# FintanH/rust-crdt

Hardware: AMD Instinct MI355X
Metric: replica-merges/sec (whole node) + achieved HBM GB/s as % of MI355X peak (higher is better)
Workload: dtype u64

## Files before the change

### rust-crdt_amd/csrc/common.hpp

```cpp
#pragma once

#include <hip/hip_runtime.h>

#include <cstdint>
#include <cstdio>
#include <algorithm>
#include <cstring>
#include <map>
#include <string>
#include <vector>

#include "crdt_gpu.h"
#include "shard_host.hpp"

namespace crdt {

using u64 = unsigned long long;
using u64x2 = unsigned long long __attribute__((ext_vector_type(2)));

constexpr int kWave = 64;

#ifndef CRDT_APPLY_WPE
#define CRDT_APPLY_WPE 0
#endif
// ... 36 lines not shown
  int map_lazyv = 1;
  int map_st = 0;
  int shagree = 0;
  int map_diag = 0;
  int rows_blocks_per_cu = 0;
  int apply_hot_slots = 8;
  int map_apply_hot = 1 << 20;
  int map_forget_vec2 = 1;
  int map_pair_reg = 1;
  int pair_rows = 256;
  int pair_ur = 8;
  int pair_occ = 1;
  int map_forget_bpc = 1;
  int mvreg_forget_bpc = 32;
  int map_pair_pf = 0;
  int map_pair_nt = 1;
  int map_pair_bpc = 64;
  int merge_flat = 1;
  int merge_flat_u = 2;
  int merge_ppl = 8;
  int stage_kb = 262144;
  int wire_walk = 1;
  int wire_fill = 1;
  int host_stream = 1;
  int apply_lane = 1;
  int apply_fence = 0;
  int orswot_apply_pf = 0;
  int orswot_apply_stg = 0;
  int orswot_apply_l2pf = 0;
  int orswot_apply_meta = 1;
  int orswot_apply_hpf = 0;
  int map_counter_dma = 0;
  int map_counter_depth = 8;
  int map_counter_kpw = 0;
  int map_counter_cs = 1;
  int map_counter_cl = 0;
  int map_orswot_cs = 0;
  int map_orswot_wide = 0;
  int map_nested_lds = 1;
  int map_apply_meta = 1;
  int map_apply_pf = 1;
  int read_bpc = 0;
  int read_unroll = 8;
  int read_nt = 1;
  int eqv_ppl = 8;
  int eqv_bpc = 32;
};

struct PendingTiming {
  std::string name;
  hipEvent_t start, stop;
};

}

struct crdt_ctx {
  int device = 0;
  hipStream_t stream = nullptr;
  int cu_count = 256;
  bool timing = false;
  crdt::Tune tune;
  std::string last_error;
  void *scratch = nullptr;
  size_t scratch_bytes = 0;
  void *dscratch = nullptr;
  size_t dscratch_bytes = 0;
  unsigned *counters = nullptr;
  size_t counters_n = 0;
  void *pinned = nullptr;
  size_t pinned_bytes = 0;
  hipEvent_t pinned_done = nullptr;
  std::map<std::string, crdt::KernelTimer> timers;
  std::vector<crdt::PendingTiming> pending;
  std::vector<hipEvent_t> free_events;
  void *comm = nullptr;
  int nranks = 1, rank = 0;
  void (*comm_destroy)(void *) = nullptr;
  void *sbuf[8] = {};
  size_t sbuf_bytes[8] = {};
  bool has_ops = false;
  crdt_comm_ops ops{};
  hipStream_t astream = nullptr;
  hipEvent_t a_main = nullptr, a_done = nullptr;
  void *a_dev = nullptr, *a_host = nullptr;
  size_t a_rows = 0;
  std::string comm_note;
  void (*comm_release)(crdt_ctx *) = nullptr;
  crdt::shard_host::PlanCache plans;
  bool chk_pending = false;
  uint64_t chk_key = 0;
  void *chk_dev = nullptr;
  uint64_t *chk_host = nullptr;
  hipEvent_t chk_ev = nullptr;
  int (*comm_check)(crdt_ctx *) = nullptr;
  int mem_kind = CRDT_MEM_DEVICE;
  hipStream_t hstream = nullptr;
  void *hbuf[2] = {};
  size_t hbuf_bytes = 0;
  void *hacc = nullptr;
  size_t hacc_bytes = 0;
  hipEvent_t hcopied[2] = {}, hfree[2] = {};
};

namespace crdt {

int fail(crdt_ctx *ctx, int code, const char *fmt, ...);
int hip_fail(crdt_ctx *ctx, hipError_t e, const char *what);
int ensure_scratch(crdt_ctx *ctx, size_t bytes);
int ensure_dscratch(crdt_ctx *ctx, size_t bytes);
int ensure_counters(crdt_ctx *ctx, size_t n);
int stage_h2d(crdt_ctx *ctx, void *dst, const void *src, size_t bytes);
int device_fill(crdt_ctx *ctx, void *dst, size_t bytes, unsigned char byte);
void timing_begin(crdt_ctx *ctx, const char *name);
void timing_end(crdt_ctx *ctx);
void timing_add_host(crdt_ctx *ctx, const char *name, double ms);

struct DefPlan {
  const size_t *def_off;
  unsigned long long G, D, M, A, Mw;
  const u64 *def_clock, *def_members;
  const u64 *out_clock;
  u64 *out_entries;
  int apply_ceiling;
  u64 *hash;
  unsigned *surv;
  unsigned *nsurv;
  uint8_t *out_keep;
  u64 *out_members;
  u64 *tkey;
  unsigned *trep;
  unsigned long long tmask;
};
int launch_deferred(crdt_ctx *ctx, const size_t *host_def_off, DefPlan q, const u64 *dev_def_off = nullptr,
                    unsigned *status = nullptr);
int stage_def_off_dev(crdt_ctx *ctx, const u64 *src, size_t *dst, size_t G, size_t D, unsigned *status,
                      unsigned *flags);

enum class Op : int { Max = 0, Or = 1 };

template <Op OP>
__device__ __forceinline__ u64 join(u64 a, u64 b) {
  if constexpr (OP == Op::Max) return a > b ? a : b;
  else return a | b;
}
template <Op OP>
__device__ __forceinline__ u64x2 join2(u64x2 a, u64x2 b) {
  u64x2 r;
  r.x = join<OP>(a.x, b.x);
  r.y = join<OP>(a.y, b.y);
  return r;
}

int lattice_lub_many(crdt_ctx *ctx, Op op, const u64 *in, size_t G, size_t R, size_t W,
                     size_t row_stride, size_t group_stride, u64 *out, size_t out_stride,
                     unsigned flags);
int lattice_merge_batch(crdt_ctx *ctx, Op op, u64 *self, const u64 *other, size_t N, size_t W,
                        size_t self_stride, size_t other_stride);
struct LubReq {
  Op op;
  const u64 *in;
  size_t G, R, W, row_stride, group_stride;
  u64 *out;
  size_t out_stride;
  unsigned flags;
};
int lattice_lub_many_multi(crdt_ctx *ctx, const LubReq *reqs, size_t n);
int lub_reqs_from_segments(crdt_ctx *ctx, const crdt_lub_segment *segs, size_t nseg, std::vector<LubReq> &reqs);

int lattice_lub_many_host(crdt_ctx *ctx, Op op, const u64 *in, size_t G, size_t R, size_t W,
                          size_t row_stride, size_t group_stride, u64 *out, size_t out_stride,
                          unsigned flags);
int lattice_merge_batch_host(crdt_ctx *ctx, Op op, u64 *self, const u64 *other, size_t N, size_t W,
                             size_t self_stride, size_t other_stride);
int lww_lub_many_dev(crdt_ctx *ctx, const u64 *marker, const u64 *val, size_t G, size_t R, size_t group_stride,
                     u64 *out_marker, u64 *out_val, u64 *first_conflict, unsigned flags);
int lww_merge_batch_dev(crdt_ctx *ctx, u64 *sm, u64 *sv, const u64 *om, const u64 *ov, size_t N, uint8_t *conflict);
int lww_lub_many_host(crdt_ctx *ctx, const u64 *marker, const u64 *val, size_t G, size_t R, size_t group_stride,
                      u64 *out_marker, u64 *out_val, u64 *first_conflict, unsigned flags);
int lww_merge_batch_host(crdt_ctx *ctx, u64 *sm, u64 *sv, const u64 *om, const u64 *ov, size_t N, uint8_t *conflict);
int orswot_lub_many_host(crdt_ctx *ctx, const crdt_orswot_batch *in, crdt_orswot_out *out);
struct OrswotJoinExtra {
  const u64 *init_clock = nullptr, *init_entries = nullptr;
  unsigned *viol = nullptr;
};
int orswot_lub_many_ex(crdt_ctx *ctx, const crdt_orswot_batch *in, crdt_orswot_out *out, const OrswotJoinExtra &ex);
int orswot_merge_batch_host(crdt_ctx *ctx, const crdt_orswot_states *self, const crdt_orswot_states *other,
                            uint32_t *status);
// ... 57 lines not shown
```

### rust-crdt_amd/csrc/ctx.cpp

```cpp
#include <cstdarg>
#include <cstdlib>

#include "common.hpp"

namespace crdt {

static thread_local std::string g_orphan_error;

int fail(crdt_ctx *ctx, int code, const char *fmt, ...) {
  char buf[512];
  va_list ap;
  va_start(ap, fmt);
  vsnprintf(buf, sizeof buf, fmt, ap);
  va_end(ap);
  if (ctx) ctx->last_error = buf;
  else g_orphan_error = buf;
  return code;
}

int hip_fail(crdt_ctx *ctx, hipError_t e, const char *what) {
  return fail(ctx, CRDT_EHIP, "%s failed: %s (%d)", what, hipGetErrorString(e), (int)e);
}

int ensure_scratch(crdt_ctx *ctx, size_t bytes) {
// ... 2 lines not shown
    (void)hipStreamSynchronize(ctx->stream);
    (void)hipFree(ctx->scratch);
    ctx->scratch = nullptr;
    ctx->scratch_bytes = 0;
  }
  size_t want = bytes < (1u << 20) ? (1u << 20) : bytes + bytes / 4;
  hipError_t e = hipMalloc(&ctx->scratch, want);
  if (e != hipSuccess) {
    ctx->scratch = nullptr;
    return fail(ctx, CRDT_ENOMEM, "scratch hipMalloc(%zu) failed: %s", want, hipGetErrorString(e));
  }
  ctx->scratch_bytes = want;
  return CRDT_OK;
}

int ensure_dscratch(crdt_ctx *ctx, size_t bytes) {
  if (bytes <= ctx->dscratch_bytes) return CRDT_OK;
  if (ctx->dscratch) {
    (void)hipStreamSynchronize(ctx->stream);
    (void)hipFree(ctx->dscratch);
    ctx->dscratch = nullptr;
    ctx->dscratch_bytes = 0;
  }
  size_t want = bytes < (1u << 16) ? (1u << 16) : bytes + bytes / 4;
  hipError_t e = hipMalloc(&ctx->dscratch, want);
  if (e != hipSuccess) {
    ctx->dscratch = nullptr;
    return fail(ctx, CRDT_ENOMEM, "dscratch hipMalloc(%zu) failed: %s", want, hipGetErrorString(e));
  }
  ctx->dscratch_bytes = want;
  return CRDT_OK;
}

int ensure_counters(crdt_ctx *ctx, size_t n) {
  if (n <= ctx->counters_n) return CRDT_OK;
  if (ctx->counters) {
    (void)hipStreamSynchronize(ctx->stream);
    (void)hipFree(ctx->counters);
    ctx->counters = nullptr;
    ctx->counters_n = 0;
  }
  size_t want = n < 16384 ? 16384 : n * 2;
  hipError_t e = hipMalloc(&ctx->counters, want * sizeof(unsigned));
  if (e != hipSuccess) {
    ctx->counters = nullptr;
    return fail(ctx, CRDT_ENOMEM, "counter hipMalloc failed: %s", hipGetErrorString(e));
  }
  ctx->counters_n = want;
  return device_fill(ctx, ctx->counters, want * sizeof(unsigned), 0);
}

int stage_h2d(crdt_ctx *ctx, void *dst, const void *src, size_t bytes) {
  if (bytes == 0) return CRDT_OK;
  if (ctx->pinned_done) {
    hipError_t e = hipEventSynchronize(ctx->pinned_done);
    if (e != hipSuccess) return hip_fail(ctx, e, "hipEventSynchronize(pinned)");
  } else {
    hipError_t e = hipEventCreateWithFlags(&ctx->pinned_done, hipEventDisableTiming);
    if (e != hipSuccess) return hip_fail(ctx, e, "hipEventCreate(pinned)");
  }
  if (bytes > ctx->pinned_bytes) {
    if (ctx->pinned) (void)hipHostFree(ctx->pinned);
    ctx->pinned = nullptr;
    ctx->pinned_bytes = 0;
    size_t want = bytes < 65536 ? 65536 : bytes * 2;
    hipError_t e = hipHostMalloc(&ctx->pinned, want, hipHostMallocDefault);
    if (e != hipSuccess) return fail(ctx, CRDT_ENOMEM, "hipHostMalloc(%zu) failed", want);
    ctx->pinned_bytes = want;
  }
  std::memcpy(ctx->pinned, src, bytes);
  hipError_t e = hipMemcpyAsync(dst, ctx->pinned, bytes, hipMemcpyHostToDevice, ctx->stream);
  if (e != hipSuccess) return hip_fail(ctx, e, "hipMemcpyAsync(staged)");
  e = hipEventRecord(ctx->pinned_done, ctx->stream);
  if (e != hipSuccess) return hip_fail(ctx, e, "hipEventRecord(pinned)");
  return CRDT_OK;
}

__global__ void fill_u64_kernel(unsigned long long *p, size_t n, unsigned long long v) {
  for (size_t i = (size_t)blockIdx.x * blockDim.x + threadIdx.x; i < n; i += (size_t)gridDim.x * blockDim.x)
    p[i] = v;
}
__global__ void fill_u8_kernel(unsigned char *p, size_t n, unsigned char v) {
  for (size_t i = (size_t)blockIdx.x * blockDim.x + threadIdx.x; i < n; i += (size_t)gridDim.x * blockDim.x)
    p[i] = v;
}

int device_fill(crdt_ctx *ctx, void *dst, size_t bytes, unsigned char byte) {
  if (bytes == 0) return CRDT_OK;
  const bool wide = (reinterpret_cast<uintptr_t>(dst) % 8 == 0) && bytes % 8 == 0;
  const size_t n = wide ? bytes / 8 : bytes;
  size_t blocks = (n + kBlock - 1) / kBlock;
  const size_t cap = (size_t)ctx->cu_count * 8;
  if (blocks > cap) blocks = cap;
  if (wide)
    hipLaunchKernelGGL(fill_u64_kernel, dim3((unsigned)blocks), dim3(kBlock), 0, ctx->stream,
                       (unsigned long long *)dst, n, 0x0101010101010101ULL * byte);
  else
    hipLaunchKernelGGL(fill_u8_kernel, dim3((unsigned)blocks), dim3(kBlock), 0, ctx->stream,
                       (unsigned char *)dst, n, byte);
  hipError_t e = hipGetLastError();
  return e == hipSuccess ? CRDT_OK : hip_fail(ctx, e, "device_fill");
}

static hipEvent_t take_event(crdt_ctx *ctx) {
  if (!ctx->free_events.empty()) {
    hipEvent_t e = ctx->free_events.back();
    ctx->free_events.pop_back();
    return e;
  }
  hipEvent_t e = nullptr;
  (void)hipEventCreate(&e);
  return e;
}

void timing_begin(crdt_ctx *ctx, const char *name) {
  if (!ctx->timing) return;
  PendingTiming p;
  p.name = name;
  p.start = take_event(ctx);
  p.stop = take_event(ctx);
  (void)hipEventRecord(p.start, ctx->stream);
  ctx->pending.push_back(p);
}

void timing_end(crdt_ctx *ctx) {
  if (!ctx->timing || ctx->pending.empty()) return;
  (void)hipEventRecord(ctx->pending.back().stop, ctx->stream);
}

void timing_add_host(crdt_ctx *ctx, const char *name, double ms) {
  if (!ctx->timing) return;
  auto &t = ctx->timers[name];
  t.total_ms += ms;
  t.launches += 1;
}

static void drain_timings(crdt_ctx *ctx) {
  for (auto &p : ctx->pending) {
    (void)hipEventSynchronize(p.stop);
    float ms = 0.f;
    if (hipEventElapsedTime(&ms, p.start, p.stop) == hipSuccess) {
      auto &t = ctx->timers[p.name];
      t.total_ms += ms;
      t.launches += 1;
    }
    ctx->free_events.push_back(p.start);
    ctx->free_events.push_back(p.stop);
  }
  ctx->pending.clear();
}

}

using namespace crdt;
// ... 68 lines not shown
      else if (k == "hot" && v >= 0 && v <= 64) ctx->tune.apply_hot_slots = v;
      else if (k == "mhot" && v >= 0) ctx->tune.map_apply_hot = v;
      else if (k == "mfv2") ctx->tune.map_forget_vec2 = v != 0;
      else if (k == "stage_kb" && v >= 4) ctx->tune.stage_kb = v;
      else if (k == "mpreg" && v >= 0 && v <= 2) ctx->tune.map_pair_reg = v;
      else if (k == "prows" && (v == 64 || v == 128 || v == 256)) ctx->tune.pair_rows = v;
      else if (k == "pur" && (v == 2 || v == 4 || v == 8)) ctx->tune.pair_ur = v;
      else if (k == "pocc" && v >= 0 && v <= 8) ctx->tune.pair_occ = v;
      else if (k == "mppl" && v >= 1 && v <= 64) ctx->tune.merge_ppl = v;
      else if (k == "mflat" && v >= 0 && v <= 16) ctx->tune.merge_flat = v;
      else if (k == "mpbpc" && v >= 1 && v <= 4096) ctx->tune.map_pair_bpc = v;
      else if (k == "mfbpc" && v >= 1 && v <= 64) ctx->tune.map_forget_bpc = v;
      else if (k == "mvfbpc" && v >= 1 && v <= 64) ctx->tune.mvreg_forget_bpc = v;
      else if (k == "eqvppl" && v >= 1 && v <= 64) ctx->tune.eqv_ppl = v;
      else if (k == "eqvbpc" && v >= 1 && v <= 4096) ctx->tune.eqv_bpc = v;
    }
    pos = end + 1;
  }
}

int crdt_ctx_create(int device, crdt_ctx **out) {
  if (!out) return fail(nullptr, CRDT_EINVAL, "crdt_ctx_create: out is NULL");
  *out = nullptr;
  int n = 0;
  hipError_t e = hipGetDeviceCount(&n);
  if (e != hipSuccess || n == 0)
    return fail(nullptr, CRDT_EHIP, "crdt_ctx_create: no HIP device (%s)", hipGetErrorString(e));
  if (device < 0 || device >= n)
    return fail(nullptr, CRDT_EINVAL, "crdt_ctx_create: device %d out of range [0,%d)", device, n);
  e = hipSetDevice(device);
  if (e != hipSuccess) return hip_fail(nullptr, e, "hipSetDevice");
  auto *ctx = new crdt_ctx();
  ctx->device = device;
  hipDeviceProp_t prop;
  if (hipGetDeviceProperties(&prop, device) == hipSuccess && prop.multiProcessorCount > 0)
    ctx->cu_count = prop.multiProcessorCount;
  if (const char *t = getenv("CRDT_TUNE")) apply_tune(ctx, t);
  *out = ctx;
  return CRDT_OK;
}

int crdt_ctx_destroy(crdt_ctx *ctx) {
  if (!ctx) return CRDT_OK;
  (void)hipSetDevice(ctx->device);
  (void)hipStreamSynchronize(ctx->stream);
  for (auto &p : ctx->pending) {
    (void)hipEventDestroy(p.start);
    (void)hipEventDestroy(p.stop);
  }
  for (auto e : ctx->free_events) (void)hipEventDestroy(e);
  if (ctx->scratch) (void)hipFree(ctx->scratch);
  if (ctx->counters) (void)hipFree(ctx->counters);
  if (ctx->dscratch) (void)hipFree(ctx->dscratch);
  if (ctx->pinned) (void)hipHostFree(ctx->pinned);
  if (ctx->pinned_done) (void)hipEventDestroy(ctx->pinned_done);
  free_stage(ctx);
  if (ctx->comm && ctx->comm_destroy) ctx->comm_destroy(ctx->comm);
  if (ctx->comm_release) ctx->comm_release(ctx);
  for (void *b : ctx->sbuf)
    if (b) (void)hipFree(b);
  delete ctx;
  return CRDT_OK;
}

int crdt_ctx_set_stream(crdt_ctx *ctx, void *hip_stream) {
  CRDT_CHECK_CTX(ctx);
  ctx->stream = reinterpret_cast<hipStream_t>(hip_stream);
  return CRDT_OK;
}

int crdt_ctx_synchronize(crdt_ctx *ctx) {
  CRDT_CHECK_CTX(ctx);
  CRDT_HIP(ctx, hipSetDevice(ctx->device));
  CRDT_HIP(ctx, hipStreamSynchronize(ctx->stream));
  if (ctx->comm_check) return ctx->comm_check(ctx);
  return CRDT_OK;
}

const char *crdt_last_error(const crdt_ctx *ctx) {
  return ctx ? ctx->last_error.c_str() : g_orphan_error.c_str();
}

const char *crdt_version(void) { return "0.8.0"; }
int crdt_abi_version(void) { return CRDT_ABI_VERSION; }
const char *crdt_build_target(void) { return "gfx950"; }

int crdt_ctx_set_timing(crdt_ctx *ctx, int enable) {
  CRDT_CHECK_CTX(ctx);
  ctx->timing = enable != 0;
  return CRDT_OK;
}

int crdt_ctx_timing(crdt_ctx *ctx, const char *name, double *total_ms, uint64_t *launches) {
  CRDT_CHECK_CTX(ctx);
  if (!name) return fail(ctx, CRDT_EINVAL, "crdt_ctx_timing: name is NULL");
  drain_timings(ctx);
  auto it = ctx->timers.find(name);
  if (total_ms) *total_ms = it == ctx->timers.end() ? 0.0 : it->second.total_ms;
  if (launches) *launches = it == ctx->timers.end() ? 0 : it->second.launches;
  return CRDT_OK;
}

int crdt_ctx_timing_reset(crdt_ctx *ctx) {
  CRDT_CHECK_CTX(ctx);
  drain_timings(ctx);
  ctx->timers.clear();
  return CRDT_OK;
}
// ... 10 lines not shown
```

### rust-crdt_amd/csrc/map.hip

```cpp
#include <type_traits>

#include "common.hpp"

namespace crdt {

struct MapPlan {
  const u64 *clock;
  long long c_rs, c_gs;
  const u64 *ec;
  long long e_rs, e_gs;
  const u64 *vclk;
  long long vc_rs, vc_gs;
  const u64 *vval;
  long long vv_rs, vv_gs;
  const size_t *def_off;
  const unsigned *def_row;
  const u64 *def_clock;
  const u64 *def_keys;
  unsigned long long G, R, K, A, V, Kw, Vout;
  u64 *o_clock, *o_ec, *o_vclk, *o_vval;
  unsigned *o_nval;
  unsigned *o_flags;
  int spec;
  int nt;
// ... 2161 lines not shown
  if (R > 0 && (!in->clock || !in->ec || (V > 0 && (!in->vclk || !in->vval))))
    return fail(ctx, CRDT_EINVAL, "map_lub_many: NULL input");
  const bool wide = A > 256 || V > 8;
  if (Vout > 64) return fail(ctx, CRDT_EUNSUPPORTED, "map_lub_many: Vout = %zu > 64", Vout);
  const bool deep = out->Vstate > 16;
  if (out->Vstate > 64) return fail(ctx, CRDT_EUNSUPPORTED, "map_lub_many: Vstate = %zu > 64", out->Vstate);
  if (deep && map_deep_lds(out->Vstate, A) > 160 * 1024)
    return fail(ctx, CRDT_EUNSUPPORTED, "map_lub_many: Vstate = %zu values of A = %zu actors need %zu bytes of LDS (> 160 KiB)",
                out->Vstate, A, map_deep_lds(out->Vstate, A));
  if (G * K > 0x7fffffffULL) return fail(ctx, CRDT_EUNSUPPORTED, "map_lub_many: G*K too large");
  if (R > 0xfffffffeULL) return fail(ctx, CRDT_EUNSUPPORTED, "map_lub_many: R too large");
  const size_t D = doff ? Ddev : (in->def_off && G > 0) ? in->def_off[G] - in->def_off[0] : 0;
  if (in->def_off && in->def_off[0] != 0) return fail(ctx, CRDT_EINVAL, "map_lub_many: def_off[0] must be 0");
  if (D > 0 && (!in->def_row || !in->def_clock || !in->def_keys || !out->def_keep || !out->def_keys))
    return fail(ctx, CRDT_EINVAL, "map_lub_many: deferred buffers missing");
  if (D > 0xffffffffULL) return fail(ctx, CRDT_EUNSUPPORTED, "map_lub_many: too many deferred");
  CRDT_HIP(ctx, hipSetDevice(ctx->device));
  const size_t Kw = (K + 63) / 64;
  const size_t want = !deep && out->Vstate > Vout ? out->Vstate : Vout;

  MapPlan p{};
  p.clock = (const u64 *)in->clock;
  p.c_rs = in->clock_rstride;
  p.c_gs = in->clock_gstride;
  p.ec = (const u64 *)in->ec;
  p.e_rs = in->ec_rstride;
  p.e_gs = in->ec_gstride;
  p.vclk = (const u64 *)in->vclk;
  p.vc_rs = in->vclk_rstride;
  p.vc_gs = in->vclk_gstride;
  p.vval = (const u64 *)in->vval;
  p.vv_rs = in->vval_rstride;
  p.vv_gs = in->vval_gstride;
  p.G = G;
  p.R = R;
  p.K = K;
  p.A = A;
  p.V = V;
  p.Kw = Kw;
  p.Vout = Vout;
  p.o_clock = (u64 *)out->clock;
  p.o_ec = (u64 *)out->ec;
  p.o_vclk = (u64 *)out->vclk;
  p.o_vval = (u64 *)out->vval;
  p.o_nval = out->nval;
  p.o_flags = out->flags;
  p.spec = ctx->tune.map_spec;
  p.nt = ctx->tune.map_nt;
  p.scan2 = ctx->tune.map_scan2 && A % 2 == 0;
  p.scan3 = ctx->tune.map_scan3;
  p.lazyv = ctx->tune.map_lazyv;
  p.batch = ctx->tune.map_batch;
  p.diag = ctx->tune.map_diag;
  if (int rc = device_fill(ctx, out->flags, G * sizeof(unsigned), 0)) return rc;
  const bool even = ((p.c_rs | p.c_gs | p.e_rs | p.e_gs | p.vc_rs | p.vc_gs) & 1) == 0;
  const bool glds = !wide && ctx->tune.map_glds && R > 0 && A <= 64 && (A & 1) == 0 && (V == 1 || V == 2) &&
                    want <= 4 && even && aligned16(p.clock) && aligned16(p.ec) && aligned16(p.vclk) &&
                    G * ((R + 7) / 8) < 0x7fffffffULL;
  const bool rs = glds && ctx->tune.map_rs && A <= 32;
  const unsigned gC = (!rs && ctx->tune.map_chunk == 8 && ctx->tune.map_ring == 4) ? 8 : 16;
  const size_t off_b = D > 0 || doff ? ((G + 1) * sizeof(size_t) + 255) / 256 * 256 : 0;
  if (glds) p.nch = (R + gC - 1) / gC;
  p.st = rs && ctx->tune.map_st && A == 32 && V == 2 && !(ctx->tune.map_sh && K % 4 == 0);
  const size_t cm_b = glds ? G * p.nch * A * sizeof(u64) : 0;
  const size_t cm_pad = (cm_b + 15) / 16 * 16, nv_b = deep && !out->nval ? G * K * sizeof(unsigned) : 0;
  if (off_b + cm_pad + nv_b > 0)
    if (int rc = ensure_scratch(ctx, off_b + cm_pad + nv_b)) return rc;
  crdt_map_out dout = *out;
  if (deep) {
    if (!dout.nval) dout.nval = reinterpret_cast<uint32_t *>(static_cast<char *>(ctx->scratch) + off_b + cm_pad);
    p.o_nval = map_deep_tag(dout.nval);
  }
  if (doff && D == 0)
    if (int rc = stage_def_off_dev(ctx, doff, (size_t *)ctx->scratch, G, 0, nullptr, out->flags)) return rc;
  if (D > 0) {
    if (doff) {
      if (int rc = stage_def_off_dev(ctx, doff, (size_t *)ctx->scratch, G, D, nullptr, out->flags)) return rc;
    } else if (int rc = stage_h2d(ctx, ctx->scratch, in->def_off, (G + 1) * sizeof(size_t))) {
      return rc;
    }
    p.def_off = reinterpret_cast<const size_t *>(ctx->scratch);
    p.def_row = in->def_row;
    p.def_clock = (const u64 *)in->def_clock;
    p.def_keys = (const u64 *)in->def_keys;
  }
  const unsigned long long blocks = G * K;
  hipError_t he;
  if (wide) {
    if (int rc = map_lub_wide(ctx, in, p.def_off, &dout, deep)) return rc;
    he = hipSuccess;
  } else {
  if (glds) {
    u64 *cm = reinterpret_cast<u64 *>(static_cast<char *>(ctx->scratch) + off_b);
    p.cmax = cm;
    timing_begin(ctx, "map_chunk_max");
    hipLaunchKernelGGL(map_chunk_max_kernel, dim3((unsigned)(G * p.nch)), dim3(64), 0, ctx->stream, p.clock,
                       p.c_rs, p.c_gs, (unsigned long long)R, (unsigned long long)A, p.nch, gC, cm);
    timing_end(ctx);
  }
  timing_begin(ctx, "map_fold");
  if (glds) {
    if (rs && ctx->tune.map_sh && A == 32 && V == 2 && K % 4 == 0)
      he = launch_map_sh(p, blocks, ctx->stream);
    else if (rs)
      he = V == 1 ? launch_map_rs<1>(p, blocks, ctx->stream) : launch_map_rs<2>(p, blocks, ctx->stream);
    else
      he = V == 1 ? launch_map_glds<1>(p, ctx->tune.map_chunk, ctx->tune.map_ring, blocks, ctx->stream)
                  : launch_map_glds<2>(p, ctx->tune.map_chunk, ctx->tune.map_ring, blocks, ctx->stream);
  } else {
    const int VI = map_vi(V, want);
    if (A <= 64) he = launch_map_vi<1>(p, VI, blocks, ctx->stream);
    else if (A <= 128) he = launch_map_vi<2>(p, VI, blocks, ctx->stream);
    else he = launch_map_vi<4>(p, VI, blocks, ctx->stream);
  }
  timing_end(ctx);
  }
  if (he != hipSuccess) return hip_fail(ctx, he, "map_fold_kernel launch");
  if (deep)
    if (int rc = map_lub_deep(ctx, in, p.def_off, &dout)) return rc;

  if (D == 0) return CRDT_OK;
  DefPlan q{};
  q.G = G;
  q.D = D;
  q.M = K;
  q.A = A;
  q.Mw = Kw;
  q.def_clock = (const u64 *)in->def_clock;
  q.def_members = (const u64 *)in->def_keys;
  q.out_clock = (const u64 *)out->clock;
  q.out_entries = nullptr;
  q.apply_ceiling = 0;
  q.out_keep = out->def_keep;
  q.out_members = (u64 *)out->def_keys;
  return launch_deferred(ctx, in->def_off, q, doff);
}

extern "C" int crdt_map_lub_many(crdt_ctx *ctx, const crdt_map_batch *in, crdt_map_out *out) {
  if (ctx && ctx->mem_kind == CRDT_MEM_HOST) return crdt::map_lub_many_host(ctx, in, out);
  CRDT_CHECK_CTX(ctx);
  if (!in || !out) return fail(ctx, CRDT_EINVAL, "map_lub_many: NULL batch/out");
  return map_lub_impl(ctx, in, nullptr, 0, out);
}

extern "C" int crdt_map_lub_many_doff(crdt_ctx *ctx, const crdt_map_batch *in, const uint64_t *def_off, size_t D,
                                      crdt_map_out *out) {
  CRDT_DEVICE_MEM_ONLY(ctx);
  CRDT_CHECK_CTX(ctx);
  if (!in || !out) return fail(ctx, CRDT_EINVAL, "map_lub_many_doff: NULL batch/out");
  if (in->def_off) return fail(ctx, CRDT_EINVAL, "map_lub_many_doff: in->def_off must be NULL");
  if (!def_off && D) return fail(ctx, CRDT_EINVAL, "map_lub_many_doff: D > 0 without def_off");
  return map_lub_impl(ctx, in, (const u64 *)def_off, D, out);
}
```

### rust-crdt_amd/csrc/orswot.hip

```cpp
#include "common.hpp"

namespace crdt {


template <int V>
struct OVec;
template <>
struct OVec<1> {
  using T = u64;
};
template <>
struct OVec<2> {
  using T = u64x2;
};

__device__ __forceinline__ u64 umax(u64 a, u64 b) { return a > b ? a : b; }

__device__ __forceinline__ u64 dot_join(u64 e1, u64 c1, u64 e2, u64 c2) {
  const u64 t0 = e1 == e2 ? e1 : 0;
  const u64 t1 = e1 > c2 ? e1 : 0;
  const u64 t2 = e2 > c1 ? e2 : 0;
  return umax(t0, umax(t1, t2));
}
__device__ __forceinline__ u64x2 dot_join(u64x2 e1, u64x2 c1, u64x2 e2, u64x2 c2) {
// ... 153 lines not shown
    if (ml == 0) part[(size_t)p.MB * kOrMPT * p.PW + cl] = c;
  }
  asm volatile("s_waitcnt vmcnt(0)" ::: "memory");
  const int bviol = __syncthreads_or(viol);
  if (l == 0) {
    __builtin_amdgcn_fence(__ATOMIC_RELEASE, "agent");
    asm volatile("s_waitcnt vmcnt(0)" ::: "memory");
    const unsigned t = __hip_atomic_fetch_add(p.cnt + u, bviol ? 0x10001u : 1u, __ATOMIC_RELAXED,
                                              __HIP_MEMORY_SCOPE_AGENT);
    const int last = (t & 0xffffu) == (unsigned)p.S - 1;
    if (last) {
      __hip_atomic_store(p.cnt + u, 0u, __ATOMIC_RELAXED, __HIP_MEMORY_SCOPE_AGENT);
      __builtin_amdgcn_fence(__ATOMIC_ACQUIRE, "agent");
      asm volatile("s_waitcnt vmcnt(0)" ::: "memory");
      if ((bviol || (t >> 16)) && p.viol) atomicOr(p.viol + g, 1u);
    }
    s_flag = last | ((bviol || (t >> 16)) ? 2 : 0);
  }
  __syncthreads();
  if (!(s_flag & 1)) return;
  if (s_flag & 2) {
    start(true);
    if (active) fold(0, p.R);
#if OR_VIOL_BALLOT
    viol |= vmask != 0;
#endif
  } else if (active) {
    c = VT(0);
#pragma unroll
    for (int j = 0; j < kOrMPT; ++j) e[j] = VT(0);
    const VT *pp = reinterpret_cast<const VT *>(p.part) + (size_t)u * p.S * slab;
    for (int k = 0; k < p.S; ++k, pp += slab) {
      const VT c2 = pp[(size_t)p.MB * kOrMPT * p.PW + cl];
#pragma unroll
      for (int j = 0; j < kOrMPT; ++j) e[j] = dot_join(e[j], c, pp[(ml + j * p.MB) * p.PW + cl], c2);
      c = umax(c, c2);
    }
  }
  store_final();
}


__device__ __forceinline__ unsigned long long group_of(const size_t *off, unsigned long long G,
                                                       unsigned long long d) {
  unsigned long long lo = 0, hi = G;
  while (hi - lo > 1) {
    const unsigned long long mid = (lo + hi) / 2;
    if (off[mid] <= d) lo = mid;
    else hi = mid;
  }
  return lo;
}

__global__ __launch_bounds__(kBlock) void orswot_deferred_kernel(DefPlan p) {
  __shared__ u64 s_hash[kBlock / kWave];
  const unsigned long long d = blockIdx.x;
  const unsigned long long g = group_of(p.def_off, p.G, d);
  const u64 *rm = p.def_clock + d * p.A;
  const u64 *cf = p.out_clock + g * p.A;
  int greater = 0;
  u64 h = 0;
  for (unsigned long long a = threadIdx.x; a < p.A; a += kBlock) {
    const u64 x = rm[a];
    greater |= x > cf[a];
    u64 z = x * 0x9E3779B97F4A7C15ULL + a;
    z = (z ^ (z >> 30)) * 0xBF58476D1CE4E5B9ULL;
    z = (z ^ (z >> 27)) * 0x94D049BB133111EBULL;
    h += z ^ (z >> 31);
  }
  const int keep = __syncthreads_or(greater);
  for (int off = kWave / 2; off > 0; off >>= 1) h += __shfl_down(h, off, kWave);
  if ((threadIdx.x & (kWave - 1)) == 0) s_hash[threadIdx.x / kWave] = h;
  const u64 *bits = p.def_members + d * p.Mw;
  u64 *E = p.out_entries + g * p.M * p.A;
  for (unsigned long long w = 0; w < p.Mw && p.apply_ceiling; ++w) {
    u64 word = bits[w];
    while (word) {
      const int bit = __builtin_ctzll(word);
      word &= word - 1;
      const unsigned long long m = w * 64 + bit;
      if (m >= p.M) break;
      u64 *row = E + m * p.A;
      for (unsigned long long a = threadIdx.x; a < p.A; a += kBlock) {
        const u64 e = row[a];
        if (e != 0 && e <= rm[a]) row[a] = 0;
      }
    }
  }
  __syncthreads();
  if (threadIdx.x == 0) {
    u64 t = 0;
    for (int w = 0; w < kBlock / kWave; ++w) t += s_hash[w];
    p.hash[d] = t;
    if (keep) p.surv[atomicAdd(p.nsurv, 1u)] = (unsigned)d;
  }
}

__device__ __forceinline__ u64 dedup_key(u64 h, unsigned long long g) {
  u64 z = h ^ ((g + 1) * 0x9E3779B97F4A7C15ULL);
  z = (z ^ (z >> 31)) * 0xD6E8FEB86659FD93ULL;
  z ^= z >> 32;
  return z ? z : 1;
}

__device__ __forceinline__ unsigned long long dedup_slot(const DefPlan &p, u64 key, bool insert, unsigned d) {
  unsigned long long t = key & p.tmask;
  while (true) {
    const u64 cur = insert ? atomicCAS(p.tkey + t, 0ull, key) : p.tkey[t];
    if (cur == key || (insert && cur == 0)) return t;
    if (!insert && cur == 0) return ~0ull;
    t = (t + 1) & p.tmask;
  }
}

__global__ __launch_bounds__(kBlock) void orswot_dedup_insert_kernel(DefPlan p) {
  const unsigned k = blockIdx.x * blockDim.x + threadIdx.x;
  const unsigned n = *p.nsurv;
  if (k >= n) return;
  const unsigned d = p.surv[k];
  const u64 key = dedup_key(p.hash[d], group_of(p.def_off, p.G, d));
  atomicMin(p.trep + dedup_slot(p, key, true, d), d);
}

__global__ __launch_bounds__(kBlock) void orswot_dedup_kernel(DefPlan p) {
  const unsigned k = blockIdx.x * blockDim.x + threadIdx.x;
  const unsigned n = *p.nsurv;
  if (k >= n) return;
  const unsigned d = p.surv[k];
  const unsigned long long g = group_of(p.def_off, p.G, d);
  const u64 key = dedup_key(p.hash[d], g);
  const unsigned long long t = dedup_slot(p, key, false, d);
  const u64 *rm = p.def_clock + (size_t)d * p.A;
  auto same = [&](unsigned d2) {
    if (d2 < p.def_off[g] || d2 >= p.def_off[g + 1]) return false;
    const u64 *rm2 = p.def_clock + (size_t)d2 * p.A;
    for (unsigned long long a = 0; a < p.A; ++a)
      if (rm[a] != rm2[a]) return false;
    return true;
  };
  unsigned rep = t == ~0ull ? d : p.trep[t];
  if (rep != d && !same(rep)) {
    rep = d;
    for (unsigned j = 0; j < n; ++j) {
      const unsigned d2 = p.surv[j];
      if (d2 < rep && p.hash[d2] == p.hash[d] && same(d2)) rep = d2;
    }
  }
  if (rep == d) p.out_keep[d] = 1;
  const u64 *src = p.def_members + (size_t)d * p.Mw;
  u64 *dst = p.out_members + (size_t)rep * p.Mw;
  for (unsigned long long w = 0; w < p.Mw; ++w)
    if (src[w]) atomicOr(dst + w, src[w]);
}

static bool al16(const void *p) { return (reinterpret_cast<uintptr_t>(p) & 15) == 0; }

__global__ __launch_bounds__(kBlock) void def_off_check_kernel(const u64 *src, size_t *dst, unsigned long long G,
                                                               unsigned long long D, unsigned *status,
                                                               unsigned *flags) {
  const unsigned long long i = (unsigned long long)blockIdx.x * kBlock + threadIdx.x;
  if (i > G) return;
  const u64 v = src[i];
  bool bad = i == 0 ? v != 0 : (i == G ? v != D : v > D);
  if (i > 0 && src[i - 1] > v) bad = true;
  dst[i] = i == 0 ? 0 : (i == G ? D : (v > D ? D : v));
  if (bad) {
    if (status) atomicOr(status, 1u);
    if (flags) {
      if (i > 0) atomicOr(flags + i - 1, 2u);
      if (i < G) atomicOr(flags + i, 2u);
    }
  }
}

int stage_def_off_dev(crdt_ctx *ctx, const u64 *src, size_t *dst, size_t G, size_t D, unsigned *status,
                      unsigned *flags) {
  const size_t n = G + 1;
  hipLaunchKernelGGL(def_off_check_kernel, dim3((unsigned)((n + kBlock - 1) / kBlock)), dim3(kBlock), 0,
                     ctx->stream, src, dst, (unsigned long long)G, (unsigned long long)D, status, flags);
  CRDT_HIP(ctx, hipGetLastError());
  return CRDT_OK;
}

int launch_deferred(crdt_ctx *ctx, const size_t *host_def_off, DefPlan q, const u64 *dev_def_off, unsigned *status) {
  const size_t G = q.G, D = q.D;
  const size_t off_b = (G + 1) * sizeof(size_t);
  size_t T = 64;
  while (T < 2 * D) T <<= 1;
  const size_t off_pad = (off_b + 255) / 256 * 256;
  const size_t need = 256 + off_pad + D * 8 + D * 4 + 64 + T * 12;
  if (int rc = ensure_dscratch(ctx, need)) return rc;
  char *base = static_cast<char *>(ctx->dscratch);
  q.nsurv = reinterpret_cast<unsigned *>(base);
  q.def_off = reinterpret_cast<const size_t *>(base + 256);
  q.hash = reinterpret_cast<u64 *>(base + 256 + off_pad);
  q.surv = reinterpret_cast<unsigned *>(q.hash + D);
  q.tkey = reinterpret_cast<u64 *>(base + ((256 + off_pad + D * 12 + 63) / 64 * 64));
  q.trep = reinterpret_cast<unsigned *>(q.tkey + T);
  q.tmask = T - 1;
  if (int rc = device_fill(ctx, q.tkey, T * 8, 0)) return rc;
  if (int rc = device_fill(ctx, q.trep, T * 4, 0xFF)) return rc;
  if (int rc = device_fill(ctx, q.nsurv, 4, 0)) return rc;
  if (dev_def_off) {
    if (int rc = stage_def_off_dev(ctx, dev_def_off, (size_t *)q.def_off, G, D, status, nullptr)) return rc;
  } else {
    int rc = stage_h2d(ctx, (void *)q.def_off, host_def_off, off_b);
    if (rc) return rc;
  }
  if (int rc = device_fill(ctx, q.out_keep, D, 0)) return rc;
  if (int rc = device_fill(ctx, q.out_members, D * q.Mw * 8, 0)) return rc;
  hipLaunchKernelGGL(orswot_deferred_kernel, dim3((unsigned)D), dim3(kBlock), 0, ctx->stream, q);
  hipLaunchKernelGGL(orswot_dedup_insert_kernel, dim3((unsigned)((D + kBlock - 1) / kBlock)), dim3(kBlock), 0,
                     ctx->stream, q);
  hipLaunchKernelGGL(orswot_dedup_kernel, dim3((unsigned)((D + kBlock - 1) / kBlock)), dim3(kBlock), 0,
                     ctx->stream, q);
  CRDT_HIP(ctx, hipGetLastError());
  return CRDT_OK;
}

}

using namespace crdt;

static int orswot_lub_impl(crdt_ctx *ctx, const crdt_orswot_batch *in, const u64 *doff, size_t Ddev,
                           crdt_orswot_out *out, unsigned *status, const OrswotJoinExtra *ex = nullptr) {
  const size_t G = in->G, R = in->R, M = in->M, A = in->A;
  if (G == 0 || A == 0) return CRDT_OK;
  if (!out->clock || (M && !out->entries)) return fail(ctx, CRDT_EINVAL, "orswot_lub_many: NULL output");
  if (R > 0 && (!in->clock || (M && !in->entries)))
    return fail(ctx, CRDT_EINVAL, "orswot_lub_many: NULL input");
  if (in->entry_mstride < A && M > 1)
    return fail(ctx, CRDT_EINVAL, "orswot_lub_many: entry_mstride < A");
  if (A > (1u << 20) || M > (1ull << 32))
    return fail(ctx, CRDT_EUNSUPPORTED, "orswot_lub_many: A or M too large");
  CRDT_HIP(ctx, hipSetDevice(ctx->device));
  const size_t D = doff ? Ddev : (in->def_off && G > 0) ? in->def_off[G] - in->def_off[0] : 0;
  if (in->def_off && in->def_off[0] != 0)
    return fail(ctx, CRDT_EINVAL, "orswot_lub_many: def_off[0] must be 0");
  const size_t Mw = (M + 63) / 64;
  if (D > 0 && (!in->def_clock || !out->def_keep || (Mw && (!in->def_members || !out->def_members))))
    return fail(ctx, CRDT_EINVAL, "orswot_lub_many: deferred buffers missing");
  if (D > 0xffffffffULL) return fail(ctx, CRDT_EUNSUPPORTED, "orswot_lub_many: too many deferred");

  if (ex && ex->viol)
    if (int rc = device_fill(ctx, ex->viol, G * 4, 0)) return rc;
  if (R == 0 && ex && ex->init_clock) {
    CRDT_HIP(ctx, hipMemcpyAsync(out->clock, ex->init_clock, G * A * 8, hipMemcpyDeviceToDevice, ctx->stream));
    if (M)
      CRDT_HIP(ctx, hipMemcpyAsync(out->entries, ex->init_entries, G * M * A * 8, hipMemcpyDeviceToDevice,
                                   ctx->stream));
  } else if (R == 0) {
    int rc = device_fill(ctx, out->clock, G * A * 8, 0);
    if (!rc && M) rc = device_fill(ctx, out->entries, G * M * A * 8, 0);
    if (rc) return rc;
  } else if (M == 0) {
    if (int rc = lattice_lub_many(ctx, Op::Max, (const u64 *)in->clock, G, R, A, in->clock_rstride,
                                  in->clock_gstride, (u64 *)out->clock, A, 0))
      return rc;
  } else {
    const bool vec2 = A % 2 == 0 && in->clock_rstride % 2 == 0 && in->clock_gstride % 2 == 0 &&
                      in->entry_mstride % 2 == 0 && in->entry_rstride % 2 == 0 &&
                      in->entry_gstride % 2 == 0 && al16(in->clock) && al16(in->entries) &&
                      al16(out->clock) && al16(out->entries) &&
                      (!ex || !ex->init_clock || (al16(ex->init_clock) && al16(ex->init_entries)));
    const int V = vec2 ? 2 : 1;
    OrPlan p{};
    p.clock = (const u64 *)in->clock;
    p.entries = (const u64 *)in->entries;
    p.c_rstride = in->clock_rstride;
    p.c_gstride = in->clock_gstride;
// ... 119 lines not shown
```

Baseline: 2.303 billion.

## Batch deferred-path fills into one prepare kernel and widen dedup per wave

Several device_fill launches and the small def_off host copy are merged into a single prepare_kernel launch that fills multiple regions and writes inline words passed as kernel arguments. The pinned staging buffer becomes a four-slot ring so stage_h2d no longer waits on the previous copy each call. The deferred ceiling-apply loop is restructured to use wave ballots and process four member rows per pass, and the dedup kernel moves from one thread to one wave per entry with lane-parallel comparisons. These changes target launch overhead and serial loops, at the cost of larger kernel arguments and more code complexity.

```diff
diff --git a/rust-crdt_amd/csrc/common.hpp b/rust-crdt_amd/csrc/common.hpp
--- a/rust-crdt_amd/csrc/common.hpp
+++ b/rust-crdt_amd/csrc/common.hpp
@@ -112,6 +112,13 @@
   hipEvent_t start, stop;
 };
 
+constexpr int kPinnedSlots = 4;
+struct PinnedSlot {
+  void *buf = nullptr;
+  size_t bytes = 0;
+  hipEvent_t done = nullptr;
+};
+
 }
 
 struct crdt_ctx {
@@ -127,9 +134,8 @@
   size_t dscratch_bytes = 0;
   unsigned *counters = nullptr;
   size_t counters_n = 0;
-  void *pinned = nullptr;
-  size_t pinned_bytes = 0;
-  hipEvent_t pinned_done = nullptr;
+  crdt::PinnedSlot pinned[crdt::kPinnedSlots];
+  unsigned pinned_next = 0;
   std::map<std::string, crdt::KernelTimer> timers;
   std::vector<crdt::PendingTiming> pending;
   std::vector<hipEvent_t> free_events;
@@ -171,6 +177,23 @@
 int ensure_counters(crdt_ctx *ctx, size_t n);
 int stage_h2d(crdt_ctx *ctx, void *dst, const void *src, size_t bytes);
 int device_fill(crdt_ctx *ctx, void *dst, size_t bytes, unsigned char byte);
+constexpr int kPrepRegions = 8;
+constexpr int kPrepWords = 32;
+struct PrepArgs {
+  void *ptr[kPrepRegions];
+  size_t bytes[kPrepRegions];
+  unsigned char byte[kPrepRegions];
+  int n = 0;
+  size_t *wdst = nullptr;
+  int nw = 0;
+  size_t w[kPrepWords];
+  void fill(void *p, size_t b, unsigned char v) {
+    if (b == 0) return;
+    ptr[n] = p, bytes[n] = b, byte[n] = v;
+    ++n;
+  }
+};
+int device_prepare(crdt_ctx *ctx, const PrepArgs &a);
 void timing_begin(crdt_ctx *ctx, const char *name);
 void timing_end(crdt_ctx *ctx);
 void timing_add_host(crdt_ctx *ctx, const char *name, double ms);
@@ -193,6 +216,9 @@
 };
 int launch_deferred(crdt_ctx *ctx, const size_t *host_def_off, DefPlan q, const u64 *dev_def_off = nullptr,
                     unsigned *status = nullptr);
+int deferred_layout(crdt_ctx *ctx, DefPlan &q, PrepArgs &pre);
+int stage_def_off_host(crdt_ctx *ctx, const size_t *src, size_t G, size_t *dst, PrepArgs &pre);
+int launch_deferred_kernels(crdt_ctx *ctx, const DefPlan &q);
 int stage_def_off_dev(crdt_ctx *ctx, const u64 *src, size_t *dst, size_t G, size_t D, unsigned *status,
                       unsigned *flags);
 
diff --git a/rust-crdt_amd/csrc/ctx.cpp b/rust-crdt_amd/csrc/ctx.cpp
--- a/rust-crdt_amd/csrc/ctx.cpp
+++ b/rust-crdt_amd/csrc/ctx.cpp
@@ -78,26 +78,28 @@
 
 int stage_h2d(crdt_ctx *ctx, void *dst, const void *src, size_t bytes) {
   if (bytes == 0) return CRDT_OK;
-  if (ctx->pinned_done) {
-    hipError_t e = hipEventSynchronize(ctx->pinned_done);
+  PinnedSlot &sl = ctx->pinned[ctx->pinned_next];
+  ctx->pinned_next = (ctx->pinned_next + 1) % kPinnedSlots;
+  if (sl.done) {
+    hipError_t e = hipEventSynchronize(sl.done);
     if (e != hipSuccess) return hip_fail(ctx, e, "hipEventSynchronize(pinned)");
   } else {
-    hipError_t e = hipEventCreateWithFlags(&ctx->pinned_done, hipEventDisableTiming);
+    hipError_t e = hipEventCreateWithFlags(&sl.done, hipEventDisableTiming);
     if (e != hipSuccess) return hip_fail(ctx, e, "hipEventCreate(pinned)");
   }
-  if (bytes > ctx->pinned_bytes) {
-    if (ctx->pinned) (void)hipHostFree(ctx->pinned);
-    ctx->pinned = nullptr;
-    ctx->pinned_bytes = 0;
+  if (bytes > sl.bytes) {
+    if (sl.buf) (void)hipHostFree(sl.buf);
+    sl.buf = nullptr;
+    sl.bytes = 0;
     size_t want = bytes < 65536 ? 65536 : bytes * 2;
-    hipError_t e = hipHostMalloc(&ctx->pinned, want, hipHostMallocDefault);
+    hipError_t e = hipHostMalloc(&sl.buf, want, hipHostMallocDefault);
     if (e != hipSuccess) return fail(ctx, CRDT_ENOMEM, "hipHostMalloc(%zu) failed", want);
-    ctx->pinned_bytes = want;
-  }
-  std::memcpy(ctx->pinned, src, bytes);
-  hipError_t e = hipMemcpyAsync(dst, ctx->pinned, bytes, hipMemcpyHostToDevice, ctx->stream);
+    sl.bytes = want;
+  }
+  std::memcpy(sl.buf, src, bytes);
+  hipError_t e = hipMemcpyAsync(dst, sl.buf, bytes, hipMemcpyHostToDevice, ctx->stream);
   if (e != hipSuccess) return hip_fail(ctx, e, "hipMemcpyAsync(staged)");
-  e = hipEventRecord(ctx->pinned_done, ctx->stream);
+  e = hipEventRecord(sl.done, ctx->stream);
   if (e != hipSuccess) return hip_fail(ctx, e, "hipEventRecord(pinned)");
   return CRDT_OK;
 }
@@ -126,6 +128,37 @@
                        (unsigned char *)dst, n, byte);
   hipError_t e = hipGetLastError();
   return e == hipSuccess ? CRDT_OK : hip_fail(ctx, e, "device_fill");
+}
+
+__global__ __launch_bounds__(kBlock) void prepare_kernel(PrepArgs a) {
+  const size_t t = (size_t)blockIdx.x * kBlock + threadIdx.x, nt = (size_t)gridDim.x * kBlock;
+  if (t < (size_t)a.nw) a.wdst[t] = a.w[t];
+  for (int r = 0; r < a.n; ++r) {
+    unsigned char *p = static_cast<unsigned char *>(a.ptr[r]);
+    const size_t b = a.bytes[r];
+    if ((reinterpret_cast<uintptr_t>(p) | b) % 8 == 0) {
+      const unsigned long long v = 0x0101010101010101ULL * a.byte[r];
+      for (size_t i = t; i < b / 8; i += nt) reinterpret_cast<unsigned long long *>(p)[i] = v;
+    } else {
+      for (size_t i = t; i < b; i += nt) p[i] = a.byte[r];
+    }
+  }
+}
+
+int device_prepare(crdt_ctx *ctx, const PrepArgs &a) {
+  if (a.n > kPrepRegions || a.nw > kPrepWords) return fail(ctx, CRDT_EINVAL, "device_prepare: too many regions / words");
+  size_t n = (size_t)a.nw;
+  for (int r = 0; r < a.n; ++r) {
+    const bool wide = (reinterpret_cast<uintptr_t>(a.ptr[r]) | a.bytes[r]) % 8 == 0;
+    n = std::max(n, wide ? a.bytes[r] / 8 : a.bytes[r]);
+  }
+  if (n == 0) return CRDT_OK;
+  size_t blocks = (n + kBlock - 1) / kBlock;
+  const size_t cap = (size_t)ctx->cu_count * 8;
+  if (blocks > cap) blocks = cap;
+  hipLaunchKernelGGL(prepare_kernel, dim3((unsigned)blocks), dim3(kBlock), 0, ctx->stream, a);
+  hipError_t e = hipGetLastError();
+  return e == hipSuccess ? CRDT_OK : hip_fail(ctx, e, "device_prepare");
 }
 
 static hipEvent_t take_event(crdt_ctx *ctx) {
@@ -300,8 +333,10 @@
   if (ctx->scratch) (void)hipFree(ctx->scratch);
   if (ctx->counters) (void)hipFree(ctx->counters);
   if (ctx->dscratch) (void)hipFree(ctx->dscratch);
-  if (ctx->pinned) (void)hipHostFree(ctx->pinned);
-  if (ctx->pinned_done) (void)hipEventDestroy(ctx->pinned_done);
+  for (auto &sl : ctx->pinned) {
+    if (sl.buf) (void)hipHostFree(sl.buf);
+    if (sl.done) (void)hipEventDestroy(sl.done);
+  }
   free_stage(ctx);
   if (ctx->comm && ctx->comm_destroy) ctx->comm_destroy(ctx->comm);
   if (ctx->comm_release) ctx->comm_release(ctx);
diff --git a/rust-crdt_amd/csrc/map.hip b/rust-crdt_amd/csrc/map.hip
--- a/rust-crdt_amd/csrc/map.hip
+++ b/rust-crdt_amd/csrc/map.hip
@@ -2237,7 +2237,6 @@
   p.lazyv = ctx->tune.map_lazyv;
   p.batch = ctx->tune.map_batch;
   p.diag = ctx->tune.map_diag;
-  if (int rc = device_fill(ctx, out->flags, G * sizeof(unsigned), 0)) return rc;
   const bool even = ((p.c_rs | p.c_gs | p.e_rs | p.e_gs | p.vc_rs | p.vc_gs) & 1) == 0;
   const bool glds = !wide && ctx->tune.map_glds && R > 0 && A <= 64 && (A & 1) == 0 && (V == 1 || V == 2) &&
                     want <= 4 && even && aligned16(p.clock) && aligned16(p.ec) && aligned16(p.vclk) &&
@@ -2256,19 +2255,34 @@
     if (!dout.nval) dout.nval = reinterpret_cast<uint32_t *>(static_cast<char *>(ctx->scratch) + off_b + cm_pad);
     p.o_nval = map_deep_tag(dout.nval);
   }
-  if (doff && D == 0)
-    if (int rc = stage_def_off_dev(ctx, doff, (size_t *)ctx->scratch, G, 0, nullptr, out->flags)) return rc;
+  PrepArgs pre{};
+  pre.fill(out->flags, G * sizeof(unsigned), 0);
+  DefPlan q{};
   if (D > 0) {
-    if (doff) {
-      if (int rc = stage_def_off_dev(ctx, doff, (size_t *)ctx->scratch, G, D, nullptr, out->flags)) return rc;
-    } else if (int rc = stage_h2d(ctx, ctx->scratch, in->def_off, (G + 1) * sizeof(size_t))) {
-      return rc;
-    }
-    p.def_off = reinterpret_cast<const size_t *>(ctx->scratch);
+    q.G = G;
+    q.D = D;
+    q.M = K;
+    q.A = A;
+    q.Mw = Kw;
+    q.def_off = reinterpret_cast<const size_t *>(ctx->scratch);
+    q.def_clock = (const u64 *)in->def_clock;
+    q.def_members = (const u64 *)in->def_keys;
+    q.out_clock = (const u64 *)out->clock;
+    q.out_entries = nullptr;
+    q.apply_ceiling = 0;
+    q.out_keep = out->def_keep;
+    q.out_members = (u64 *)out->def_keys;
+    if (int rc = deferred_layout(ctx, q, pre)) return rc;
+    if (!doff)
+      if (int rc = stage_def_off_host(ctx, in->def_off, G, (size_t *)ctx->scratch, pre)) return rc;
+    p.def_off = q.def_off;
     p.def_row = in->def_row;
     p.def_clock = (const u64 *)in->def_clock;
     p.def_keys = (const u64 *)in->def_keys;
   }
+  if (int rc = device_prepare(ctx, pre)) return rc;
+  if (doff)
+    if (int rc = stage_def_off_dev(ctx, doff, (size_t *)ctx->scratch, G, D, nullptr, out->flags)) return rc;
   const unsigned long long blocks = G * K;
   hipError_t he;
   if (wide) {
@@ -2305,20 +2319,7 @@
     if (int rc = map_lub_deep(ctx, in, p.def_off, &dout)) return rc;
 
   if (D == 0) return CRDT_OK;
-  DefPlan q{};
-  q.G = G;
-  q.D = D;
-  q.M = K;
-  q.A = A;
-  q.Mw = Kw;
-  q.def_clock = (const u64 *)in->def_clock;
-  q.def_members = (const u64 *)in->def_keys;
-  q.out_clock = (const u64 *)out->clock;
-  q.out_entries = nullptr;
-  q.apply_ceiling = 0;
-  q.out_keep = out->def_keep;
-  q.out_members = (u64 *)out->def_keys;
-  return launch_deferred(ctx, in->def_off, q, doff);
+  return launch_deferred_kernels(ctx, q);
 }
 
 extern "C" int crdt_map_lub_many(crdt_ctx *ctx, const crdt_map_batch *in, crdt_map_out *out) {
diff --git a/rust-crdt_amd/csrc/orswot.hip b/rust-crdt_amd/csrc/orswot.hip
--- a/rust-crdt_amd/csrc/orswot.hip
+++ b/rust-crdt_amd/csrc/orswot.hip
@@ -229,6 +229,7 @@
   return lo;
 }
 
+constexpr int kDefU = 4;
 __global__ __launch_bounds__(kBlock) void orswot_deferred_kernel(DefPlan p) {
   __shared__ u64 s_hash[kBlock / kWave];
   const unsigned long long d = blockIdx.x;
@@ -248,19 +249,48 @@
   const int keep = __syncthreads_or(greater);
   for (int off = kWave / 2; off > 0; off >>= 1) h += __shfl_down(h, off, kWave);
   if ((threadIdx.x & (kWave - 1)) == 0) s_hash[threadIdx.x / kWave] = h;
-  const u64 *bits = p.def_members + d * p.Mw;
-  u64 *E = p.out_entries + g * p.M * p.A;
-  for (unsigned long long w = 0; w < p.Mw && p.apply_ceiling; ++w) {
-    u64 word = bits[w];
-    while (word) {
-      const int bit = __builtin_ctzll(word);
-      word &= word - 1;
-      const unsigned long long m = w * 64 + bit;
-      if (m >= p.M) break;
-      u64 *row = E + m * p.A;
-      for (unsigned long long a = threadIdx.x; a < p.A; a += kBlock) {
-        const u64 e = row[a];
-        if (e != 0 && e <= rm[a]) row[a] = 0;
+  if (p.apply_ceiling) {
+    const bool per_wave = p.A <= (unsigned long long)kWave;
+    const int wv = __builtin_amdgcn_readfirstlane((int)(threadIdx.x / kWave));
+    const u64 wmask = per_wave ? 0xFFFFull << (16 * wv) : ~0ull;
+    const unsigned long long a0 = per_wave ? threadIdx.x % kWave : threadIdx.x;
+    const unsigned long long astep = per_wave ? kWave : kBlock;
+    const u64 *bits = p.def_members + d * p.Mw;
+    u64 *E = p.out_entries + g * p.M * p.A;
+    const unsigned lane = threadIdx.x % kWave;
+    for (unsigned long long w0 = 0; w0 < p.Mw; w0 += kWave) {
+      const u64 mine = (w0 + lane < p.Mw ? bits[w0 + lane] : 0) & wmask;
+      u64 todo = __ballot(mine != 0);
+      while (todo) {
+        const int wl = __builtin_ctzll(todo);
+        todo &= todo - 1;
+        const unsigned long long w = w0 + wl;
+        u64 word = ((u64)__builtin_amdgcn_readlane((unsigned)(mine >> 32), wl) << 32) |
+                   __builtin_amdgcn_readlane((unsigned)mine, wl);
+        while (word) {
+          unsigned long long row[kDefU];
+          bool ok[kDefU];
+#pragma unroll
+          for (int j = 0; j < kDefU; ++j) {
+            row[j] = 0;
+            ok[j] = false;
+            if (word) {
+              const unsigned long long m = w * 64 + __builtin_ctzll(word);
+              word &= word - 1;
+              ok[j] = m < p.M;
+              if (ok[j]) row[j] = m * p.A;
+            }
+          }
+          for (unsigned long long a = a0; a < p.A; a += astep) {
+            const u64 r = rm[a];
+            u64 e[kDefU];
+#pragma unroll
+            for (int j = 0; j < kDefU; ++j) e[j] = E[row[j] + a];
+#pragma unroll
+            for (int j = 0; j < kDefU; ++j)
+              if (ok[j] && e[j] != 0 && e[j] <= r) E[row[j] + a] = 0;
+          }
+        }
       }
     }
   }
@@ -300,7 +330,8 @@
 }
 
 __global__ __launch_bounds__(kBlock) void orswot_dedup_kernel(DefPlan p) {
-  const unsigned k = blockIdx.x * blockDim.x + threadIdx.x;
+  const unsigned lane = threadIdx.x % kWave;
+  const unsigned long long k = (unsigned long long)blockIdx.x * (kBlock / kWave) + threadIdx.x / kWave;
   const unsigned n = *p.nsurv;
   if (k >= n) return;
   const unsigned d = p.surv[k];
@@ -311,9 +342,9 @@
   auto same = [&](unsigned d2) {
     if (d2 < p.def_off[g] || d2 >= p.def_off[g + 1]) return false;
     const u64 *rm2 = p.def_clock + (size_t)d2 * p.A;
-    for (unsigned long long a = 0; a < p.A; ++a)
-      if (rm[a] != rm2[a]) return false;
-    return true;
+    bool ne = false;
+    for (unsigned long long a = lane; a < p.A; a += kWave) ne |= rm[a] != rm2[a];
+    return __ballot(ne) == 0;
   };
   unsigned rep = t == ~0ull ? d : p.trep[t];
   if (rep != d && !same(rep)) {
@@ -323,10 +354,10 @@
       if (d2 < rep && p.hash[d2] == p.hash[d] && same(d2)) rep = d2;
     }
   }
-  if (rep == d) p.out_keep[d] = 1;
+  if (rep == d && lane == 0) p.out_keep[d] = 1;
   const u64 *src = p.def_members + (size_t)d * p.Mw;
   u64 *dst = p.out_members + (size_t)rep * p.Mw;
-  for (unsigned long long w = 0; w < p.Mw; ++w)
+  for (unsigned long long w = lane; w < p.Mw; w += kWave)
     if (src[w]) atomicOr(dst + w, src[w]);
 }
 
@@ -359,7 +390,7 @@
   return CRDT_OK;
 }
 
-int launch_deferred(crdt_ctx *ctx, const size_t *host_def_off, DefPlan q, const u64 *dev_def_off, unsigned *status) {
+int deferred_layout(crdt_ctx *ctx, DefPlan &q, PrepArgs &pre) {
   const size_t G = q.G, D = q.D;
   const size_t off_b = (G + 1) * sizeof(size_t);
   size_t T = 64;
@@ -369,30 +400,53 @@
   if (int rc = ensure_dscratch(ctx, need)) return rc;
   char *base = static_cast<char *>(ctx->dscratch);
   q.nsurv = reinterpret_cast<unsigned *>(base);
-  q.def_off = reinterpret_cast<const size_t *>(base + 256);
+  if (!q.def_off) q.def_off = reinterpret_cast<const size_t *>(base + 256);
   q.hash = reinterpret_cast<u64 *>(base + 256 + off_pad);
   q.surv = reinterpret_cast<unsigned *>(q.hash + D);
   q.tkey = reinterpret_cast<u64 *>(base + ((256 + off_pad + D * 12 + 63) / 64 * 64));
   q.trep = reinterpret_cast<unsigned *>(q.tkey + T);
   q.tmask = T - 1;
-  if (int rc = device_fill(ctx, q.tkey, T * 8, 0)) return rc;
-  if (int rc = device_fill(ctx, q.trep, T * 4, 0xFF)) return rc;
-  if (int rc = device_fill(ctx, q.nsurv, 4, 0)) return rc;
-  if (dev_def_off) {
-    if (int rc = stage_def_off_dev(ctx, dev_def_off, (size_t *)q.def_off, G, D, status, nullptr)) return rc;
-  } else {
-    int rc = stage_h2d(ctx, (void *)q.def_off, host_def_off, off_b);
-    if (rc) return rc;
-  }
-  if (int rc = device_fill(ctx, q.out_keep, D, 0)) return rc;
-  if (int rc = device_fill(ctx, q.out_members, D * q.Mw * 8, 0)) return rc;
+  if (pre.n + 5 > kPrepRegions) return fail(ctx, CRDT_EINVAL, "deferred_layout: no room in the prepare launch");
+  pre.fill(q.tkey, T * 8, 0);
+  pre.fill(q.trep, T * 4, 0xFF);
+  pre.fill(q.nsurv, 4, 0);
+  pre.fill(q.out_keep, D, 0);
+  pre.fill(q.out_members, D * q.Mw * 8, 0);
+  return CRDT_OK;
+}
+
+int stage_def_off_host(crdt_ctx *ctx, const size_t *src, size_t G, size_t *dst, PrepArgs &pre) {
+  if (G + 1 <= (size_t)kPrepWords && pre.nw == 0) {
+    pre.wdst = dst;
+    pre.nw = (int)(G + 1);
+    std::memcpy(pre.w, src, (G + 1) * sizeof(size_t));
+    return CRDT_OK;
+  }
+  return stage_h2d(ctx, dst, src, (G + 1) * sizeof(size_t));
+}
+
+int launch_deferred_kernels(crdt_ctx *ctx, const DefPlan &q) {
+  const size_t D = q.D;
+  constexpr size_t wpb = kBlock / kWave;
   hipLaunchKernelGGL(orswot_deferred_kernel, dim3((unsigned)D), dim3(kBlock), 0, ctx->stream, q);
   hipLaunchKernelGGL(orswot_dedup_insert_kernel, dim3((unsigned)((D + kBlock - 1) / kBlock)), dim3(kBlock), 0,
                      ctx->stream, q);
-  hipLaunchKernelGGL(orswot_dedup_kernel, dim3((unsigned)((D + kBlock - 1) / kBlock)), dim3(kBlock), 0,
-                     ctx->stream, q);
+  hipLaunchKernelGGL(orswot_dedup_kernel, dim3((unsigned)((D + wpb - 1) / wpb)), dim3(kBlock), 0, ctx->stream, q);
   CRDT_HIP(ctx, hipGetLastError());
   return CRDT_OK;
+}
+
+int launch_deferred(crdt_ctx *ctx, const size_t *host_def_off, DefPlan q, const u64 *dev_def_off, unsigned *status) {
+  PrepArgs pre{};
+  q.def_off = nullptr;
+  if (int rc = deferred_layout(ctx, q, pre)) return rc;
+  if (dev_def_off) {
+    if (int rc = stage_def_off_dev(ctx, dev_def_off, (size_t *)q.def_off, q.G, q.D, status, nullptr)) return rc;
+  } else if (int rc = stage_def_off_host(ctx, host_def_off, q.G, (size_t *)q.def_off, pre)) {
+    return rc;
+  }
+  if (int rc = device_prepare(ctx, pre)) return rc;
+  return launch_deferred_kernels(ctx, q);
 }
 
 }
```

New measurement: 2.302 billion. About the same (-0.0%).
